# kspalaiologos/modern-rzip

Measured on AMD Instinct MI355X. Metric: rzip-stage GiB/s (mrzip -n), higher is better.
Workload: dtype u8; 1 GPU; tar-64G: rzip stage of mrzip -L7 on a 64 GiB synthetic tar (60 % text members, 25 % noise, 15 % exact duplicates, 512-byte aligned; BASELINE configs[2], the largest single-GPU configuration), one chunk per GPU, input resident in HBM; level=7, chunk_bytes_per_gpu=68719476736, streams=1, mode=streams

## Files before the change

### modern-rzip_amd/csrc/mrz_seq_deep.hip

```cpp
#ifndef MRZ_DEEP_WAVES
#define MRZ_DEEP_WAVES 8
#endif
#define MRZ_SEQ_WAVES MRZ_DEEP_WAVES
#include "mrz_seq_common.h"
#include <cstddef>

#ifndef MRZ_DEEP_LANES
#define MRZ_DEEP_LANES 256
#endif
#ifndef MRZ_DEEP_GROUP
#define MRZ_DEEP_GROUP 8
#endif
#define MRZ_DEEP_THREADS (64 * MRZ_DEEP_WAVES)
#ifdef __HIP_DEVICE_COMPILE__
#define MRZ_DEEP_WAIT() asm volatile("s_waitcnt vmcnt(0)" ::: "memory")
#else
#define MRZ_DEEP_WAIT() ((void)0)
#endif
#define MRZ_DEEP_MAP 2048
#define MRZ_DEEP_CW_WORDS 32
#define MRZ_DEEP_XW 192

enum { MRZ_DK_NONE = 255, MRZ_DK_EMPTY = 0, MRZ_DK_OVER = 1, MRZ_DK_DISPLACE = 2, MRZ_DK_EVICT = 3 };
#define MRZ_DF_INS 1
#define MRZ_DF_CPLX 2
#define MRZ_DF_STALE 4
#define MRZ_DF_FE2 8
#define MRZ_DS_COOP 1
#define MRZ_DS_CONFLICT 2
#define MRZ_DS_CULLED 4
#define MRZ_DS_NOCULL 8

struct mrz_deep_recs {
    int64_t q[MRZ_DEEP_LANES], t[MRZ_DEEP_LANES];
    int64_t occ_t[MRZ_DEEP_LANES], occ_off[MRZ_DEEP_LANES];
    int64_t old_t[MRZ_DEEP_LANES], old_t2[MRZ_DEEP_LANES];
    int64_t cp_scan[MRZ_DEEP_LANES];
    int64_t alt_old_t[MRZ_DEEP_LANES];
    int alt_w[MRZ_DEEP_LANES];
    int h[MRZ_DEEP_LANES], fe[MRZ_DEEP_LANES], w[MRZ_DEEP_LANES], h2[MRZ_DEEP_LANES], w2[MRZ_DEEP_LANES];
    unsigned short xw_seen[MRZ_DEEP_LANES];
    unsigned char kind[MRZ_DEEP_LANES], kind2[MRZ_DEEP_LANES], nsame[MRZ_DEEP_LANES], flags[MRZ_DEEP_LANES];
    unsigned char alt_kind[MRZ_DEEP_LANES];
    int same_slot[MRZ_DEEP_LANES][MRZ_SMAX];
    int64_t same_off[MRZ_DEEP_LANES][MRZ_SMAX];
    unsigned short raw[MRZ_DEEP_LANES][MRZ_SMAX];
};

struct mrz_deep_lds {
    mrz_lead lead;
    int ctl[16];
    int wsum[MRZ_DEEP_WAVES], wsum2[MRZ_DEEP_WAVES], wmin[MRZ_DEEP_WAVES], wmin2[MRZ_DEEP_WAVES], wmin3[MRZ_DEEP_WAVES];
    int n_rescan;
    mrz_deep_recs R;
    int idx[MRZ_DEEP_LANES];
    int cmin[MRZ_DEEP_LANES];
    int cpos[MRZ_DEEP_LANES];
    int xw_n;
    int xw_slot[MRZ_DEEP_XW];
    unsigned short rescan_list[MRZ_DEEP_LANES];
    unsigned smap_key[MRZ_DEEP_MAP];
    int smap_lane[MRZ_DEEP_MAP];
    unsigned long long tmap_key[MRZ_DEEP_MAP];
    int tmap_lane[MRZ_DEEP_MAP];
    mrz_u64 cw[MRZ_DEEP_CW_WORDS];
    int cwcum[MRZ_DEEP_CW_WORDS + 1];
#ifdef MRZ_SEQ_STATS
    int64_t stat[MRZ_ST_N], stat_unused[MRZ_ST_N];
#endif
    mrz_coop_lds coop;
};

__device__ __forceinline__ bool mrz_deep_ranges_meet(int a, int la, int b, int lb, int smask) {
    return la > 0 && lb > 0 && ((((b - a) & smask) < la) || (((a - b) & smask) < lb));
}

__device__ static unsigned mrz_deep_probe_raw(const uint8_t *__restrict__ buf, int64_t q, int64_t op, int64_t end) {
    if (op >= q) return 0;
    int64_t maxf = end - q;
    if (maxf < 0) maxf = 0;
    const int64_t last_ok = end + (MRZ_MIN_MATCH - 16);
    uint4 fa[4], fb[4], ba[4], bb[4];
#pragma unroll
    for (int j = 0; j < 4; j++) {
        int64_t pa = q + j * 16, pb = op + j * 16;
        pa = pa < last_ok ? pa : last_ok;
        pb = pb < last_ok ? pb : last_ok;
        fa[j] = mrz_ld16(buf + pa);
        fb[j] = mrz_ld16(buf + pb);
        int64_t ra = q - (j + 1) * 16, rb = op - (j + 1) * 16;
        ra = ra > 0 ? ra : 0;
        rb = rb > 0 ? rb : 0;
        ba[j] = mrz_ld16(buf + ra);
        bb[j] = mrz_ld16(buf + rb);
    }
    int rawf;
    {
        const int d0 = mrz_first_diff16_bf(fa[0], fb[0]), d1 = mrz_first_diff16_bf(fa[1], fb[1]);
        const int d2 = mrz_first_diff16_bf(fa[2], fb[2]), d3 = mrz_first_diff16_bf(fa[3], fb[3]);
        rawf = d0 < 16 ? d0 : 16 + (d1 < 16 ? d1 : 16 + (d2 < 16 ? d2 : 16 + d3));
// ... 220 lines not shown
                fe = (sb + fe_idx) & smask;
                fe2 = fe_idx < 63 && ((m_empty >> (fe_idx + 1)) & 1);
            }
        }
    }
    if (nsame > MRZ_SMAX) cplx = true;
    if (kind == MRZ_DK_EVICT && max_chain > MRZ_SMAX) cplx = true;
    int h2 = 0, w2 = -1, kind2 = MRZ_DK_NONE;
    int64_t old_t2 = 0;
    if (kind == MRZ_DK_DISPLACE && !cplx) {
        const int rank2 = mrz_ones_rank(occ_t);
        h2 = (int)(occ_t & C.slot_mask);
        int round2 = 0;
        bool done = false;
        for (int grp = 0; !done; grp++) {
            if (grp >= max_groups) {
                cplx = true;
                break;
            }
            mrz_slot e[MRZ_DEEP_GROUP];
            const int s0 = h2 + grp * (64 * MRZ_DEEP_GROUP) + lane;
#pragma unroll
            for (int g = 0; g < MRZ_DEEP_GROUP; g++) e[g] = tab[(s0 + g * 64) & smask];
#pragma unroll
            for (int g = 0; g < MRZ_DEEP_GROUP; g++) {
                if (done) continue;
                const int sb = s0 - lane + g * 64;
                const bool empty = (e[g].off | e[g].t) == 0;
                const bool due = !empty && (e[g].t & better) != better;
                const bool low = !empty && !due && mrz_ones_rank(e[g].t) < rank2;
                const mrz_u64 m_empty = __ballot(empty), m_due = __ballot(due), m_low = __ballot(low);
                const mrz_u64 m_stop = m_empty | m_due | m_low;
                const int ks = m_stop ? __ffsll((long long)m_stop) - 1 : 64;
                const int nq = __popcll(__ballot(!empty && !due && !low && e[g].t == occ_t) & mrz_low_mask(ks));
                if (round2 + nq >= max_chain) {
                    cplx = true;
                    done = true;
                } else if (ks < 64) {
                    if ((m_low >> ks) & 1)
                        cplx = true;
                    else {
                        w2 = (sb + ks) & smask;
                        kind2 = ((m_empty >> ks) & 1) ? MRZ_DK_EMPTY : MRZ_DK_OVER;
                        if (kind2 == MRZ_DK_OVER) old_t2 = mrz_bcast64(e[g].t, ks);
                    }
                    done = true;
                } else
                    round2 += nq;
            }
        }
    }
    const int ns = nsame < MRZ_SMAX ? nsame : MRZ_SMAX;
    if (ns > nsame0) {
        MRZ_WAVE_SYNC();
        if (lane >= nsame0 && lane < ns) S->R.raw[i][lane] = (unsigned short)mrz_deep_probe_raw(buf, q, S->R.same_off[i][lane], C.end);
    }
    if (lane == 0) {
        S->R.h[i] = h;
        S->R.fe[i] = fe;
        S->R.w[i] = w;
        S->R.kind[i] = (unsigned char)(kind < 0 ? MRZ_DK_NONE : kind);
        S->R.h2[i] = h2;
        S->R.w2[i] = w2;
        S->R.kind2[i] = (unsigned char)kind2;
        S->R.occ_t[i] = occ_t;
        S->R.occ_off[i] = occ_off;
        S->R.old_t[i] = old_t;
        S->R.old_t2[i] = old_t2;
        S->R.alt_w[i] = (cplx || kind == MRZ_DK_DISPLACE || kind == MRZ_DK_EVICT || insert_kept) ? -1 : alt_w;
        S->R.alt_kind[i] = (unsigned char)alt_kind;
        S->R.alt_old_t[i] = alt_old_t;
        S->R.nsame[i] = (unsigned char)ns;
        S->R.flags[i] = (unsigned char)((ins ? MRZ_DF_INS : 0) | (cplx ? MRZ_DF_CPLX : 0) | (fe2 ? MRZ_DF_FE2 : 0));
        if (!cont) {
            S->R.cp_scan[i] = clean_ptr;
            S->R.xw_seen[i] = (unsigned short)xw_n;
        }
    }
}

#ifndef MRZ_DEEP_SCANNERS
#define MRZ_DEEP_SCANNERS 63
#endif
#ifndef MRZ_DEEP_HELP_MIN
#define MRZ_DEEP_HELP_MIN 48
#endif

struct mrz_deep_shared {
    unsigned long long seq;
    unsigned long long quit;
    unsigned long long n_ok;
    unsigned long long xcc_plus1;
    unsigned long long pad0[12];
    long long nb, nscan, better, tag_mask, clean_ptr, xw_n;
    long long pad1[10];
    unsigned long long done;
    unsigned long long pad2[15];
    mrz_deep_recs R;
};

#ifdef __HIP_DEVICE_COMPILE__
#define MRZ_DEEP_ACQUIRE() __builtin_amdgcn_fence(__ATOMIC_ACQUIRE, "agent")
#define MRZ_DEEP_RELEASE() __builtin_amdgcn_fence(__ATOMIC_RELEASE, "agent")
#define MRZ_DEEP_XCC_ID() (__builtin_amdgcn_s_getreg(20 | (0 << 6) | (3 << 11)) & 15)
#else
#define MRZ_DEEP_ACQUIRE() ((void)0)
#define MRZ_DEEP_RELEASE() ((void)0)
#define MRZ_DEEP_XCC_ID() 0
#endif

__device__ __forceinline__ void mrz_deep_rec_copy(mrz_deep_recs *dst, const mrz_deep_recs *src, int i) {
    dst->occ_t[i] = src->occ_t[i];
    dst->occ_off[i] = src->occ_off[i];
    dst->old_t[i] = src->old_t[i];
    dst->old_t2[i] = src->old_t2[i];
    dst->cp_scan[i] = src->cp_scan[i];
    dst->alt_old_t[i] = src->alt_old_t[i];
    dst->alt_w[i] = src->alt_w[i];
    dst->alt_kind[i] = src->alt_kind[i];
    dst->h[i] = src->h[i];
    dst->fe[i] = src->fe[i];
    dst->w[i] = src->w[i];
    dst->h2[i] = src->h2[i];
    dst->w2[i] = src->w2[i];
    dst->xw_seen[i] = src->xw_seen[i];
    dst->kind[i] = src->kind[i];
    dst->kind2[i] = src->kind2[i];
    dst->flags[i] = src->flags[i];
    const int ns = src->nsame[i];
    dst->nsame[i] = (unsigned char)ns;
    for (int k = 0; k < ns; k++) {
        dst->same_slot[i][k] = src->same_slot[i][k];
        dst->same_off[i][k] = src->same_off[i][k];
        dst->raw[i][k] = src->raw[i][k];
    }
}


__device__ static void mrz_deep_scan_helper(const mrz_cfg &C, mrz_deep_lds *S, mrz_deep_shared *G, int tid, int lane, int wave) {
    if (tid == 0) {
        long long spins = 0;
        unsigned long long x = 0;
        while ((x = __hip_atomic_load(&G->xcc_plus1, __ATOMIC_RELAXED, __HIP_MEMORY_SCOPE_AGENT)) == 0 &&
               !__hip_atomic_load(&G->quit, __ATOMIC_RELAXED, __HIP_MEMORY_SCOPE_AGENT) && spins++ < (1ll << 24))
            __builtin_amdgcn_s_sleep(8);
        int ticket = -1;
        if (x != 0)
            ticket = (int)__hip_atomic_fetch_add(&G->n_ok, 1ull, __ATOMIC_RELAXED, __HIP_MEMORY_SCOPE_AGENT);
        S->ctl[0] = ticket;
    }
    __syncthreads();
    const int ticket = mrz_uni(S->ctl[0]);
    if (ticket < 0 || ticket >= MRZ_DEEP_SCANNERS) return;
    const int me = ticket + 1;
    unsigned long long seen = 0;
    while (true) {
        if (tid == 0) {
            long long spins = 0;
            unsigned long long sq = 0;
            int v = 1;
            while (true) {
                sq = __hip_atomic_load(&G->seq, __ATOMIC_RELAXED, __HIP_MEMORY_SCOPE_AGENT);
                if (sq != seen) break;
                if (__hip_atomic_load(&G->quit, __ATOMIC_RELAXED, __HIP_MEMORY_SCOPE_AGENT) || spins++ > MRZ_HELPER_SPIN_LIMIT) {
                    v = 0;
                    break;
                }
                __builtin_amdgcn_s_sleep(2);
            }
            MRZ_DEEP_ACQUIRE();
            S->ctl[1] = v;
            S->lead.p = (int64_t)sq;
        }
        __syncthreads();
        if (!mrz_uni(S->ctl[1])) return;
        seen = (unsigned long long)mrz_uni64(S->lead.p);
        const int nb = (int)G->nb, nscan = (int)G->nscan, xw_n = (int)G->xw_n;
        const int64_t better = G->better, tag_mask = G->tag_mask, clean_ptr = G->clean_ptr;
        int mine_n = 0;
        if (me < nscan) {
            for (int i = me + tid * nscan; i < nb; i += nscan * MRZ_DEEP_THREADS) {
                S->R.q[i] = G->R.q[i];
                S->R.t[i] = G->R.t[i];
            }
            __syncthreads();
            int k = 0;
            for (int i = me; i < nb; i += nscan, k++)
                if (k % MRZ_DEEP_WAVES == wave) mrz_deep_scan(C, S, i, better, tag_mask, clean_ptr, xw_n, lane);
            mine_n = k;
            __syncthreads();
            for (int i = me + tid * nscan; i < nb; i += nscan * MRZ_DEEP_THREADS) mrz_deep_rec_copy(&G->R, &S->R, i);
            MRZ_DEEP_WAIT();
        }
        __syncthreads();
        if (tid == 0 && mine_n) {
            MRZ_DEEP_RELEASE();
            __hip_atomic_fetch_add(&G->done, (unsigned long long)mine_n, __ATOMIC_RELEASE, __HIP_MEMORY_SCOPE_AGENT);
        }
    }
}

__device__ static __attribute__((noinline)) bool mrz_deep_coop(const mrz_cfg &C, mrz_lead &L, mrz_coop_lds *B, int64_t t,
                                                               int lane, int64_t *stat) {
    return mrz_seq_candidate(C, L, B, t, lane, stat);
}

__device__ static __attribute__((noinline)) bool mrz_deep_candidate_rec(const mrz_cfg &C, mrz_lead &L, mrz_deep_lds *S, int i, int *xw_n, int lane,
                                              int64_t *stat) {
    mrz_coop_lds *B = &S->coop;
    const int64_t q = mrz_uni64(S->R.q[i]), t = mrz_uni64(S->R.t[i]);
    const int ns = mrz_uni((int)S->R.nsame[i]);
    const int f = mrz_uni((int)S->R.flags[i]);
    int64_t mlen = 0, m_off = 0, m_rev = 0;
    L.p = q;
    if (ns) {
        if (lane < ns) {
            const int64_t op = S->R.same_off[i][lane];
            B->same_off[lane] = op;
            int64_t ml, rv;
            bool lng;
            mrz_lane_match_len(C.buf, q, op, C.end, L.last_match, &ml, &rv, &lng);
            B->pair_res[lane] = lng ? -1 : (int)((ml << 8) | rv);
        }
        MRZ_WAVE_SYNC();
        int xh = 0, xm = 0;
        if (!mrz_resolve_entries(C, L, B, q, ns, lane, stat, &mlen, &m_off, &m_rev, &xh, &xm)) return false;
        L.tag_hits += xh;
        L.tag_misses += xm;
    }
    int nx = *xw_n;
    if (f & MRZ_DF_INS) {
        const int kind = mrz_uni((int)S->R.kind[i]);
        L.inserts++;
        L.count++;
        int ws = mrz_uni(S->R.w[i]);
        if (kind == MRZ_DK_OVER)
            L.count--;
        else if (kind == MRZ_DK_EVICT) {
            L.count--;
            ws = mrz_uni(S->R.same_slot[i][(int)L.victim_round]);
            L.victim_round = L.victim_round + 1 == C.max_chain ? 0 : L.victim_round + 1;
        } else if (kind == MRZ_DK_DISPLACE) {
            const int w2 = mrz_uni(S->R.w2[i]);
            if (mrz_uni((int)S->R.kind2[i]) == MRZ_DK_OVER) L.count--;
            if (lane == 0) {
                mrz_slot oc;
                oc.off = S->R.occ_off[i];
                oc.t = S->R.occ_t[i];
                C.tab[w2] = oc;
                S->xw_slot[nx] = w2;
            }
            nx++;
        }
        if (lane == 0) {
            mrz_slot nw;
            nw.off = q;
            nw.t = t;
            C.tab[ws] = nw;
            S->xw_slot[nx] = ws;
        }
        nx++;
        if (L.count > C.limit) {
            MRZ_DEEP_WAIT();
            mrz_cull_one(C, L, lane);
            if (lane == 0) S->xw_slot[nx] = (int)L.clean_ptr;
            nx++;
        }
    }
    *xw_n = nx;
    return mrz_select_emit(C, L, mlen, m_off, m_rev, lane);
}

__device__ __forceinline__ int mrz_deep_incl(int v, int *ws, int lane, int wave, int *total) {
    const int incl = mrz_wave_incl_sum(v, lane);
    if (lane == 63) ws[wave] = incl;
    __syncthreads();
    int add = 0, tot = 0;
#pragma unroll
    for (int w = 0; w < MRZ_DEEP_WAVES; w++) {
        const int x = ws[w];
        tot += x;
        if (w < wave) add += x;
// ... 5 lines not shown
__device__ __forceinline__ int mrz_deep_first(bool flag, int *wm, int lane, int wave, int tid, int none) {
    const mrz_u64 m = __ballot(flag);
    if (lane == 0) wm[wave] = m ? wave * 64 + (__ffsll((long long)m) - 1) : none;
    __syncthreads();
    int r = none;
#pragma unroll
    for (int w = 0; w < MRZ_DEEP_WAVES; w++) r = wm[w] < r ? wm[w] : r;
    return r;
}

__global__ __launch_bounds__(MRZ_DEEP_THREADS) void mrz_seq_deep_kernel(mrz_seq_args a, mrz_deep_shared *G, int scanners) {
#ifdef MRZ_EMU_LDS_PER_BLOCK
    static mrz_deep_lds deep_all[1 + 15];
    mrz_deep_lds *S = &deep_all[(blockIdx.x / 8) % (1 + 15)];
#else
    __shared__ mrz_deep_lds deep;
    mrz_deep_lds *S = &deep;
#endif
    const int tid = (int)threadIdx.x;
    const int lane = tid & 63;
    const int wave = mrz_uni(tid >> 6);
    mrz_seq_state *st = a.st;
    if (st->finished || st->error) return;
    const int xcd = a.xcd & 7;
    const int bx = (int)blockIdx.x;
    const bool is_seq = bx == xcd;
#ifdef MRZ_EMU_LDS_PER_BLOCK
    const bool is_scanner = G != nullptr && !is_seq && bx % 8 == xcd && bx / 8 >= 1 && bx / 8 <= scanners && bx / 8 <= MRZ_DEEP_SCANNERS;
#else
    const bool is_scanner = G != nullptr && !is_seq && (bx < xcd ? bx : bx - 1) < scanners && scanners <= MRZ_DEEP_SCANNERS;
#endif
#if MRZ_HELPER_WGS > 0
    if (!is_seq && !is_scanner) {
        if (a.gmailbox) mrz_helper_wg(a.buf, (mrz_gmailbox *)a.gmailbox);
        return;
    }
#else
    if (!is_seq && !is_scanner) return;
#endif
    mrz_cfg C;
    C.buf = a.buf;
    C.tab = a.tab;
    C.events = a.events;
    C.st = st;
    C.end = st->end;
    C.limit = st->limit;
    C.max_chain = st->max_chain;
    C.slot_mask = st->slot_mask;
    C.nslots = st->slot_mask + 1;
    C.event_cap = st->event_cap;
    C.ev_base = st->ev_base;
    C.gmb = (mrz_gmailbox *)a.gmailbox;
    unsigned long long gseq = 0;
    C.gseq = &gseq;
    int gnw = 0;
    C.gnw = &gnw;
    C.n_helpers = a.n_helpers;
    int64_t farm_hint = 0;
    C.farm_hint = &farm_hint;
    int long_seen = 0;
    C.long_seen = &long_seen;
    C.mb = nullptr;
    C.mb_seq = nullptr;
    mrz_cands K;
    K.cand = a.cand;
    K.tile_off = a.tile_off;
    K.bitmap = a.bitmap;
    K.seg_start = st->seg_start;
    K.seg_end = st->seg_end;
    K.n = st->n_cand;
    if (is_scanner) {
        mrz_deep_scan_helper(C, S, G, tid, lane, wave);
        return;
    }
    if (K.seg_end <= K.seg_start) {
        if (tid == 0 && G) __hip_atomic_store(&G->quit, 1ull, __ATOMIC_RELAXED, __HIP_MEMORY_SCOPE_AGENT);
#if MRZ_HELPER_WGS > 0
        if (tid == 0 && C.gmb) mrz_g_storeu(&C.gmb->quit, 1ull);
#endif
        return;
    }
    if (tid == 0 && G) __hip_atomic_store(&G->xcc_plus1, (unsigned long long)MRZ_DEEP_XCC_ID() + 1ull, __ATOMIC_RELAXED, __HIP_MEMORY_SCOPE_AGENT);
    unsigned long long batch_seq = 0;
    const int64_t lim = (C.end < K.seg_end - 1) ? C.end : K.seg_end - 1;
    const int smask = (int)C.slot_mask;
    const int max_chain = (int)C.max_chain;
#ifdef MRZ_SEQ_STATS
    for (int k = tid; k < MRZ_ST_N; k += MRZ_DEEP_THREADS) S->stat[k] = 0;
    __syncthreads();
    int64_t *stat = tid == 0 ? S->stat : S->stat_unused;
#else
    int64_t *stat = nullptr;
#endif

    mrz_lead L;
    L.p = st->p;
    L.cur_p = st->cur_p;
    L.cur_ofs = st->cur_ofs;
    L.cur_len = st->cur_len;
    L.last_match = st->last_match;
    L.min_mask = st->min_mask;
    L.tag_mask = st->tag_mask;
    L.count = st->count;
    L.clean_ptr = st->clean_ptr;
    L.victim_round = st->victim_round;
    L.n_events = st->n_events;
    L.inserts = st->inserts;
    L.tag_hits = st->tag_hits;
    L.tag_misses = st->tag_misses;
    L.last_len = 0;
    L.mbytes = 0;
    const int64_t hint_p0 = L.p, hint_ev0 = L.n_events;

    int64_t ci;
    {
        int64_t pos = L.p + 1;
        if (pos < K.seg_start) pos = K.seg_start;
        ci = mrz_cand_lower_bound(K, pos, lane);
    }
    bool ok = true;
    PROF_T0();
#ifdef MRZ_SEQ_PROFILE
    const int64_t launch_t0 = (int64_t)__builtin_amdgcn_s_memtime();
#endif
    ST_ADD(MRZ_ST_D_LAUNCHES, 1);
    while (ok && ci < K.n && L.p < lim) {
        PROF_T0R();
        const int64_t better = (L.min_mask << 1) | 1;
        const bool loose = L.tag_mask != better;
        int64_t my_q = 0, my_t = 0;
        bool live = false;
        if (ci + tid < K.n) {
            const mrz_cand c = K.cand[ci + tid];
            my_q = c.off;
            my_t = c.t;
            live = c.off > L.p && c.off <= lim && (c.t & L.min_mask) == L.min_mask;
        }
        int total;
        const int incl = mrz_deep_incl(live ? 1 : 0, S->wsum, lane, wave, &total);
        const int at = incl - 1;
        if (live && at < MRZ_DEEP_LANES) {
            S->R.q[at] = my_q;
            S->R.t[at] = my_t;
            S->idx[at] = (int)(ci + tid);
        }
        const int nb = total < MRZ_DEEP_LANES ? total : MRZ_DEEP_LANES;
        int64_t n_examined = K.n - ci < MRZ_DEEP_THREADS ? K.n - ci : MRZ_DEEP_THREADS;
        __syncthreads();
        if (total > MRZ_DEEP_LANES) n_examined = (int64_t)S->idx[MRZ_DEEP_LANES - 1] + 1 - ci;
        if (nb == 0) {
            ci += n_examined;
            __syncthreads();
            continue;
        }
        ST_ADD(MRZ_ST_D_BATCHES, 1);
        ST_ADD(MRZ_ST_D_LANES, nb);
        PROF_ADD(MRZ_ST_D_T_FORM);
        if (!loose) {
            int nscan = 1;
            if (G && nb >= MRZ_DEEP_HELP_MIN) {
                int nh = (int)mrz_uni64((int64_t)__hip_atomic_load(&G->n_ok, __ATOMIC_RELAXED, __HIP_MEMORY_SCOPE_AGENT));
                if (nh > MRZ_DEEP_SCANNERS) nh = MRZ_DEEP_SCANNERS;
                if (nh > scanners) nh = scanners;
                nscan = 1 + nh;
            }
            int helper_lanes = 0;
            if (nscan > 1) {
                if (tid < nb) {
                    G->R.q[tid] = S->R.q[tid];
                    G->R.t[tid] = S->R.t[tid];
                }
                if (tid == 0) {
                    G->nb = nb;
                    G->nscan = nscan;
                    G->better = better;
                    G->tag_mask = L.tag_mask;
                    G->clean_ptr = L.clean_ptr;
                    G->xw_n = 0;
                    __hip_atomic_store(&G->done, 0ull, __ATOMIC_RELAXED, __HIP_MEMORY_SCOPE_AGENT);
                }
                MRZ_DEEP_WAIT();
                __syncthreads();
                batch_seq++;
                if (tid == 0) {
                    MRZ_DEEP_RELEASE();
                    __hip_atomic_store(&G->seq, batch_seq, __ATOMIC_RELEASE, __HIP_MEMORY_SCOPE_AGENT);
                }
                helper_lanes = nb - (nb + nscan - 1) / nscan;
            }
            {
                int k = 0;
                for (int i = 0; i < nb; i += nscan, k++)
                    if (k % MRZ_DEEP_WAVES == wave) mrz_deep_scan(C, S, i, better, L.tag_mask, L.clean_ptr, 0, lane);
            }
            if (nscan > 1) {
                if (tid == 0) {
                    long long spins = 0;
                    while (__hip_atomic_load(&G->done, __ATOMIC_ACQUIRE, __HIP_MEMORY_SCOPE_AGENT) < (unsigned long long)helper_lanes &&
                           spins++ < (1ll << 26))
                        __builtin_amdgcn_s_sleep(1);
                    S->ctl[6] = spins < (1ll << 26) ? 1 : 0;
                    MRZ_DEEP_ACQUIRE();
                }
                __syncthreads();
                if (!mrz_uni(S->ctl[6])) {
                    if (tid == 0) C.st->error = 7;
                    ok = false;
                } else if (tid < nb && tid % nscan != 0)
                    mrz_deep_rec_copy(&S->R, &G->R, tid);
            }
        }
        __syncthreads();
        PROF_ADD(MRZ_ST_D_T_SCAN);
        for (int k = tid; k < MRZ_DEEP_MAP; k += MRZ_DEEP_THREADS) {
            S->smap_key[k] = 0u;
            S->smap_lane[k] = 0x7fffffff;
            S->tmap_key[k] = 0ull;
            S->tmap_lane[k] = 0x7fffffff;
        }
        __syncthreads();
        int next = 0;
        bool cut = false;
        int xw_n = 0;
        while (next < nb && !cut && ok) {
            const int i = tid;
            const bool mine = i >= next && i < nb;
            const int round_start = next;
            int coop_lane = -1;
            bool use_record = false;
            if (loose || L.cur_len > 0) {
                coop_lane = next;
            } else {
                const int64_t cw_base = L.clean_ptr;
                const bool load_cw = L.count + (nb - next) > C.limit;
                constexpr int CW_PER_WAVE = (MRZ_DEEP_CW_WORDS + MRZ_DEEP_WAVES - 1) / MRZ_DEEP_WAVES;
                mrz_slot cwe[CW_PER_WAVE];
#pragma unroll
                for (int b = 0; b < CW_PER_WAVE; b++) {
                    cwe[b].off = 0;
                    cwe[b].t = 0;
                    const int wi = b * MRZ_DEEP_WAVES + wave;
                    const int64_t slot = cw_base + (int64_t)wi * 64 + lane;
                    if (load_cw && wi < MRZ_DEEP_CW_WORDS && slot < C.nslots) cwe[b] = C.tab[slot];
                }
                const int f = mine ? S->R.flags[i] : 0;
                const bool ins = mine && (f & MRZ_DF_INS), cplx = mine && (f & MRZ_DF_CPLX);
                const int kind = mine ? S->R.kind[i] : MRZ_DK_NONE, kind2 = mine ? S->R.kind2[i] : MRZ_DK_NONE;
                const int64_t q = mine ? S->R.q[i] : 0, t = mine ? S->R.t[i] : 0;
                const int w = mine ? S->R.w[i] : -1, w2 = mine ? S->R.w2[i] : -1, fe = mine ? S->R.fe[i] : -1;
                const int h = mine ? S->R.h[i] : 0, h2 = mine ? S->R.h2[i] : 0;
                const int64_t occ_t = mine ? S->R.occ_t[i] : 0;
                const bool wr_w = ins && !cplx && (kind == MRZ_DK_EMPTY || kind == MRZ_DK_OVER || kind == MRZ_DK_DISPLACE);
                const bool wr_w2 = ins && !cplx && kind == MRZ_DK_DISPLACE;
                if (ins && !cplx) {
                    if (wr_w) mrz_deep_smap_put(S, w, i);
                    if (wr_w2) mrz_deep_smap_put(S, w2, i);
                    mrz_deep_tmap_put(S, t, i);
                    if (kind == MRZ_DK_OVER) mrz_deep_tmap_put(S, S->R.old_t[i], i);
                    if (kind == MRZ_DK_DISPLACE) {
                        mrz_deep_tmap_put(S, occ_t, i);
                        if (kind2 == MRZ_DK_OVER) mrz_deep_tmap_put(S, S->R.old_t2[i], i);
                    }
                }
                __syncthreads();
                int res = 0, res_x = -1;
                int w_e = w, kind_e = kind, fe_e = fe;
                if (mine && !cplx && !(f & MRZ_DF_STALE) && kind != MRZ_DK_DISPLACE) {
                    const int m_t = mrz_deep_tmap_get(S, t);
                    const int m_fe = mrz_deep_smap_get(S, fe);
                    const int m_w = wr_w ? mrz_deep_smap_get(S, w) : 0x7fffffff;
                    const bool c_w = wr_w && m_w < i, c_fe = m_fe < i;
                    if (m_t >= i && (c_w || c_fe)) {
                        bool can = true;
                        const int aw = S->R.alt_w[i], ak = S->R.alt_kind[i];
                        if (c_w) {
                            const int x = m_w;
                            res_x = x;
                            const int kx = S->R.kind[x];
                            can = aw >= 0 && S->R.w[x] == w && (kx == MRZ_DK_EMPTY || kx == MRZ_DK_OVER) &&
                                  mrz_ones_rank(S->R.t[x]) >= mrz_ones_rank(t);
                            res |= 1;
                            if (kind == MRZ_DK_EMPTY) res |= 2;
                        }
                        if (c_fe && !(res & 2)) {
                            can = can && (f & MRZ_DF_FE2) && !((res & 1) && ak == MRZ_DK_EMPTY);
                            res |= 2;
                        }
                        if (!can) res = 0;
                    }
                    if (res & 1) {
                        w_e = S->R.alt_w[i];
                        kind_e = S->R.alt_kind[i];
// ... 293 lines not shown
                                             : mrz_deep_coop(C, L, &S->coop, t, lane, stat);
                        ST_ADD(MRZ_ST_D_COOP, 1);
                        ST_ADD(MRZ_ST_D_COOP_REC, rec ? 1 : 0);
                        const bool same_masks = L.min_mask == mm0 && L.tag_mask == tm0;
                        const int nwr = rec ? 0 : mrz_uni(S->coop.n_written);
                        const int64_t cs = rec ? -1 : mrz_uni64(S->coop.cull_slot);
                        const bool room = nx + nwr + 1 <= MRZ_DEEP_XW;
                        if (rec)
                            nx = nx_rec;
                        else if (okc && same_masks && room && !loose) {
                            if (lane < nwr) S->xw_slot[nx + lane] = (int)S->coop.pend_h[lane];
                            nx += nwr;
                            if (cs >= 0) {
                                if (lane == 0) S->xw_slot[nx] = (int)cs;
                                nx++;
                            }
                        }
                        verdict = !okc ? 3 : ((same_masks && (room || loose) && L.p >= q) ? 1 : 2);
                        if (!(loose && verdict == 1)) break;
                        int j = cl + 1;
                        while (j < nb && mrz_uni64(S->R.q[j]) <= L.p) j++;
                        if (j >= nb) break;
                        cl = j;
                    }
                    if (lane == 0) {
                        S->lead = L;
                        S->ctl[0] = verdict;
                        S->ctl[5] = nx;
                    }
                    MRZ_DEEP_WAIT();
                }
                __syncthreads();
                L = S->lead;
                xw_n = mrz_uni(S->ctl[5]);
                const int v = mrz_uni(S->ctl[0]);
                if (v == 3) ok = false;
                if (v == 2) cut = true;
                {
                    const int i = tid;
                    const int nf = mrz_deep_first(i > coop_lane && i < nb && S->R.q[i] > L.p, S->wmin3, lane, wave, tid, nb);
                    next = nf;
                }
                PROF_ADD(MRZ_ST_D_T_COOP);
            }
        }
        if (ok) {
            if (cut || L.p > mrz_uni64(S->R.q[nb - 1])) {
                int64_t pos = L.p + 1;
                if (pos < K.seg_start) pos = K.seg_start;
                ci = mrz_cand_lower_bound(K, pos, lane);
            } else
                ci += n_examined;
        }
        __syncthreads();
    }
    if (ok && ci >= K.n && L.p < lim) L.p = lim;
#ifdef MRZ_SEQ_PROFILE
    stat[MRZ_ST_D_T_TOTAL] += (int64_t)__builtin_amdgcn_s_memtime() - launch_t0;
#endif
    if (tid == 0) {
        if (G) __hip_atomic_store(&G->quit, 1ull, __ATOMIC_RELAXED, __HIP_MEMORY_SCOPE_AGENT);
#if MRZ_HELPER_WGS > 0
        if (C.gmb) mrz_g_storeu(&C.gmb->quit, 1ull);
#endif
        st->p = L.p;
        st->cur_p = L.cur_p;
        st->cur_ofs = L.cur_ofs;
        st->cur_len = L.cur_len;
        st->last_match = L.last_match;
        st->min_mask = L.min_mask;
        st->tag_mask = L.tag_mask;
        st->count = L.count;
        st->clean_ptr = L.clean_ptr;
        st->victim_round = L.victim_round;
        st->n_events = L.n_events;
        st->inserts = L.inserts;
        st->tag_hits = L.tag_hits;
        st->tag_misses = L.tag_misses;
        st->finished = L.p >= C.end ? 1 : 0;
        st->hint_positions = L.p - hint_p0;
        st->hint_events = L.n_events - hint_ev0;
        st->hint_matched = L.mbytes;
#ifdef MRZ_SEQ_STATS
        for (int k = 0; k < MRZ_ST_N; k++) st->prof[k] += stat[k];
#endif
    }
}

extern "C" hipError_t mrz_launch_sequencer_deep(hipStream_t stream, const uint8_t *buf, mrz_slot *tab, const mrz_cand *cand,
                                                const int *tile_off, const mrz_u64 *bitmap, mrz_event *events,
                                                mrz_seq_state *st, void *gmailbox, int n_helpers, int xcd, void *deep_shared,
                                                int scanners) {
    mrz_seq_args a;
    a.buf = buf;
    a.tab = tab;
    a.cand = cand;
    a.tile_off = tile_off;
    a.bitmap = bitmap;
    a.events = events;
    a.st = st;
    a.gmailbox = gmailbox;
    a.xcd = xcd & 7;
    a.deep_bits = 0;
#if MRZ_HELPER_WGS == 0
    n_helpers = 0;
#endif
    if (n_helpers > MRZ_HELPER_WGS) n_helpers = MRZ_HELPER_WGS;
    if (n_helpers < 0 || !gmailbox) n_helpers = 0;
    a.n_helpers = n_helpers;
    if (gmailbox) {
        hipError_t e = hipMemsetAsync(gmailbox, 0, sizeof(mrz_gmailbox), stream);
        if (e != hipSuccess) return e;
    }
    if (scanners < 0 || !deep_shared) scanners = 0;
    if (scanners > MRZ_DEEP_SCANNERS) scanners = MRZ_DEEP_SCANNERS;
    unsigned grid = (unsigned)(1 + a.n_helpers);
    if (grid < (unsigned)(a.xcd + 1)) grid = (unsigned)(a.xcd + 1);
#ifdef MRZ_EMU_LDS_PER_BLOCK
    if (scanners > 0) {
        grid = (unsigned)(8 * scanners + a.xcd + 1);
        emu::request_coresident();
    }
#else
    if (scanners > a.n_helpers / 2) scanners = a.n_helpers / 2;
    while (scanners > 0 && grid < (unsigned)(scanners + 2)) scanners--;
#endif
    if (deep_shared) {
        hipError_t e = hipMemsetAsync(deep_shared, 0, offsetof(mrz_deep_shared, R), stream);
        if (e != hipSuccess) return e;
    }
    hipLaunchKernelGGL(mrz_seq_deep_kernel, dim3(grid), dim3(MRZ_DEEP_THREADS), 0, stream, a, (mrz_deep_shared *)deep_shared,
                       scanners);
    return hipGetLastError();
}

extern "C" size_t mrz_seq_deep_shared_size(void) { return sizeof(mrz_deep_shared); }
```

### modern-rzip_amd/csrc/mrz_seq_stats.h

```cpp
#pragma once
#include "mrz_common.h"

#define MRZ_SEQ_STATS_LIST(X) \
    X(BATCHES, "batches") X(FORMED, "formed") X(COMMITTED, "committed") X(SEGMENTS, "segments") \
    X(EMITS, "emits") X(BACKJUMP, "backjump") X(REWALK, "rewalk") X(LONGRES, "longres") X(SEQ, "seq_cands") \
    X(CUT_CPLX, "cut_cplx") X(CUT_OVERFLOW, "cut_overflow") X(SKIPOUT, "skipout") X(CONF0, "conf0") \
    X(PAIRS, "pairs") X(T_FORM, "t_form") X(T_WALK, "t_walk") X(T_CONF, "t_conf") X(T_PAIRS, "t_pairs") \
    X(T_LOOP, "t_loop") X(T_REWALK, "t_rewalk") X(T_LONG, "t_long") X(T_SEQ, "t_seq") X(FARMED, "farmed") \
    X(L_POST, "l_post") X(L_STRIPE, "l_stripe") X(L_BWD, "l_bwd") X(L_WAIT, "l_wait") X(L_ROUNDS, "l_rounds") \
    X(F_POST, "f_post") X(F_WAIT, "f_wait") X(F_FOLD, "f_fold") X(S_TAB, "s_tab") X(S_PAIR, "s_pair") \
    X(S_INS, "s_ins") X(OVL, "ovl") X(OVL_OK, "ovl_ok") X(X_WALK, "x_walk") X(X_CASC, "x_casc") \
    X(X_POOL, "x_pool") X(X_WIN, "x_win") X(X_SAME, "x_same") X(C_WIN, "c_win") X(C_EVICT, "c_evict") \
    X(C_DEEP, "c_deep") X(C_MANY, "c_many") X(C_FAIL, "c_fail") X(C_TIE, "c_tie") X(C_NW, "c_nw") \
    X(T_OVL, "t_ovl") X(H_PRE, "h_pre") X(H_CAND, "h_cand") X(H_POST, "h_post") X(T_SCAN, "t_scan") \
    X(T_FOLD, "t_fold") X(T_COMMIT, "t_commit") X(REPREP, "reprep") X(W_STALE, "w_stale") X(W_DROP, "w_drop") \
    X(RESET, "reset") X(T_TURN, "t_turn") X(T_PREP, "t_prep") X(T_PRECOMMIT, "t_precommit") X(E_MASK, "e_mask") \
    X(E_CULL, "e_cull") X(E_XW, "e_xw") X(E_INWIN, "e_inwin") X(E_WINDOW, "e_window") X(E_BULK, "e_bulk") \
    X(E_MORE, "e_more") X(T_PC_CW, "t_pc_cw") X(T_PC_LOG, "t_pc_log") X(T_PC_BEST, "t_pc_best") \
    X(T_PC_BULK, "t_pc_bulk") X(T_TURNWORK, "t_turnwork") X(T_SNAP, "t_snap") X(REBULK, "rebulk") \
     \
    X(BATCH_LANES, "batch_lanes") X(CUT_LONG, "cut_long") X(CUT_WALK, "cut_walk") \
    X(CUT_CONFLICT, "cut_conflict") X(CUT_CULL, "cut_cull") X(BATCH_EMITS, "batch_emits") \
    X(CUT_CASCADE, "cut_cascade") X(BATCH_FORMED, "batch_formed") X(T_WALK2, "t_walk2") X(T_SCANS, "t_scans") \
    X(T_CONFLICT, "t_conflict") X(T_WINDOW, "t_window") \
     \
    X(D_BATCHES, "d_batches") X(D_LANES, "d_lanes") X(D_ROUNDS, "d_rounds") X(D_RESCANNED, "d_rescanned") \
    X(D_COOP, "d_coop") X(D_T_FORM, "d_t_form") X(D_T_SCAN, "d_t_scan") X(D_T_COMMIT, "d_t_commit") \
    X(D_T_RESCAN, "d_t_rescan") X(D_T_TOTAL, "d_t_total") X(D_LAUNCHES, "d_launches") X(D_T_COOP, "d_t_coop") \
    X(D_COOP_REC, "d_coop_rec") X(D_RESOLVED, "d_resolved") X(D_S_COOP, "d_s_coop") \
    X(D_S_CONFLICT, "d_s_conflict") X(D_S_CULLED, "d_s_culled") X(D_S_NOCULL, "d_s_nocull") \
    X(D_S_STALE, "d_s_stale") X(D_C_OVER_ALT, "d_c_over_alt") X(D_C_OVER_NOALT, "d_c_over_noalt") \
    X(D_C_EMPTY, "d_c_empty") X(D_C_DISPLACE, "d_c_displace") X(D_C_OTHER, "d_c_other")

#define MRZ_ST_ENUM(id, name) MRZ_ST_##id,
enum { MRZ_SEQ_STATS_LIST(MRZ_ST_ENUM) MRZ_ST_N };
#undef MRZ_ST_ENUM
static_assert(MRZ_ST_N <= (int)(sizeof(((mrz_seq_state *)0)->prof) / sizeof(int64_t)), "mrz_seq_state.prof holds the counters");
```

Baseline: 6.362 GiB/s.

## Hand off deep-scan records as packed 16-byte granules with stamped jobs and unfenced counters

Scanner helpers now pack each scanned record into an array-of-structs of 16-byte granules and write it right after scanning, using buffer stores with a cache-coherence bit instead of a field-by-field struct-of-arrays copy after a barrier. The leader pulls those granules back with vectorised loads. Job parameters go out as a single stamped 16-byte word so helpers can detect a stale job, and the done counter becomes cumulative, which lets the agent-scope release/acquire fences be dropped on both sides. This is meant to cut handoff latency and fence cost per batch. It relies on the SC1 buffer semantics for coherence in place of explicit fences, which is a correctness risk if those semantics do not hold. Optional profiling counters are also added.

```diff
diff --git a/modern-rzip_amd/csrc/mrz_seq_deep.hip b/modern-rzip_amd/csrc/mrz_seq_deep.hip
--- a/modern-rzip_amd/csrc/mrz_seq_deep.hip
+++ b/modern-rzip_amd/csrc/mrz_seq_deep.hip
@@ -16,6 +16,20 @@
 #define MRZ_DEEP_WAIT() asm volatile("s_waitcnt vmcnt(0)" ::: "memory")
 #else
 #define MRZ_DEEP_WAIT() ((void)0)
+#endif
+#ifdef MRZ_SEQ_PROFILE
+#define DPROF_T0() int64_t dprof_t0 = (int64_t)__builtin_amdgcn_s_memtime()
+#define DPROF_T0R() dprof_t0 = (int64_t)__builtin_amdgcn_s_memtime()
+#define DPROF_ADD(acc)                                               \
+    do {                                                             \
+        const int64_t now__ = (int64_t)__builtin_amdgcn_s_memtime(); \
+        (acc) += now__ - dprof_t0;                                   \
+        dprof_t0 = now__;                                            \
+    } while (0)
+#else
+#define DPROF_T0()
+#define DPROF_T0R()
+#define DPROF_ADD(acc)
 #endif
 #define MRZ_DEEP_MAP 2048
 #define MRZ_DEEP_CW_WORDS 32
@@ -402,9 +416,34 @@
 #ifndef MRZ_DEEP_SCANNERS
 #define MRZ_DEEP_SCANNERS 63
 #endif
+#define MRZ_DEEP_STAMP_RETRIES (1 << 20)
 #ifndef MRZ_DEEP_HELP_MIN
 #define MRZ_DEEP_HELP_MIN 48
 #endif
+
+#define MRZ_DEEP_REC_HDR 5
+#define MRZ_DEEP_REC_GRANULES (MRZ_DEEP_REC_HDR + MRZ_SMAX)
+struct mrz_deep_rec_ent {
+    int64_t same_off;
+    int same_slot;
+    unsigned short raw, pad;
+};
+struct __attribute__((aligned(16))) mrz_deep_rec {
+    int64_t occ_t, occ_off;
+    int64_t old_t, old_t2;
+    int64_t cp_scan, alt_old_t;
+    int alt_w, h, fe, w;
+    int h2, w2;
+    unsigned short xw_seen;
+    unsigned char kind, kind2, nsame, flags, alt_kind, pad;
+    mrz_deep_rec_ent ent[MRZ_SMAX];
+};
+static_assert(sizeof(mrz_deep_rec_ent) == 16 && sizeof(mrz_deep_rec) == 16 * MRZ_DEEP_REC_GRANULES, "records travel as 16-byte granules");
+
+struct __attribute__((aligned(16))) mrz_deep_stamp {
+    unsigned long long job_seq;
+    int nb, nscan;
+};
 
 struct mrz_deep_shared {
     unsigned long long seq;
@@ -412,12 +451,17 @@
     unsigned long long n_ok;
     unsigned long long xcc_plus1;
     unsigned long long pad0[12];
-    long long nb, nscan, better, tag_mask, clean_ptr, xw_n;
+    mrz_deep_stamp stamp;
+    long long better, tag_mask, clean_ptr, xw_n;
     long long pad1[10];
     unsigned long long done;
     unsigned long long pad2[15];
-    mrz_deep_recs R;
+    int64_t q[MRZ_DEEP_LANES], t[MRZ_DEEP_LANES];
+    mrz_deep_rec rec[MRZ_DEEP_LANES];
 };
+static_assert(offsetof(mrz_deep_shared, stamp) % 128 == 0 && offsetof(mrz_deep_shared, done) % 128 == 0 &&
+                  offsetof(mrz_deep_shared, q) % 128 == 0 && offsetof(mrz_deep_shared, rec) % 16 == 0,
+              "the polled words, the job and the counter have lines of their own; granules are aligned");
 
 #ifdef __HIP_DEVICE_COMPILE__
 #define MRZ_DEEP_ACQUIRE() __builtin_amdgcn_fence(__ATOMIC_ACQUIRE, "agent")
@@ -429,33 +473,136 @@
 #define MRZ_DEEP_XCC_ID() 0
 #endif
 
-__device__ __forceinline__ void mrz_deep_rec_copy(mrz_deep_recs *dst, const mrz_deep_recs *src, int i) {
-    dst->occ_t[i] = src->occ_t[i];
-    dst->occ_off[i] = src->occ_off[i];
-    dst->old_t[i] = src->old_t[i];
-    dst->old_t2[i] = src->old_t2[i];
-    dst->cp_scan[i] = src->cp_scan[i];
-    dst->alt_old_t[i] = src->alt_old_t[i];
-    dst->alt_w[i] = src->alt_w[i];
-    dst->alt_kind[i] = src->alt_kind[i];
-    dst->h[i] = src->h[i];
-    dst->fe[i] = src->fe[i];
-    dst->w[i] = src->w[i];
-    dst->h2[i] = src->h2[i];
-    dst->w2[i] = src->w2[i];
-    dst->xw_seen[i] = src->xw_seen[i];
-    dst->kind[i] = src->kind[i];
-    dst->kind2[i] = src->kind2[i];
-    dst->flags[i] = src->flags[i];
-    const int ns = src->nsame[i];
-    dst->nsame[i] = (unsigned char)ns;
-    for (int k = 0; k < ns; k++) {
-        dst->same_slot[i][k] = src->same_slot[i][k];
-        dst->same_off[i][k] = src->same_off[i][k];
-        dst->raw[i][k] = src->raw[i][k];
-    }
-}
-
+__device__ static __attribute__((noinline)) uint4 mrz_deep_rec_granule(const mrz_deep_recs *R, int i, int g) {
+    if (g < 3) {
+        const int64_t a = g == 0 ? R->occ_t[i] : g == 1 ? R->old_t[i] : R->cp_scan[i];
+        const int64_t b = g == 0 ? R->occ_off[i] : g == 1 ? R->old_t2[i] : R->alt_old_t[i];
+        return make_uint4((uint32_t)(uint64_t)a, (uint32_t)((uint64_t)a >> 32), (uint32_t)(uint64_t)b, (uint32_t)((uint64_t)b >> 32));
+    }
+    if (g == 3) return make_uint4((uint32_t)R->alt_w[i], (uint32_t)R->h[i], (uint32_t)R->fe[i], (uint32_t)R->w[i]);
+    if (g == 4)
+        return make_uint4((uint32_t)R->h2[i], (uint32_t)R->w2[i],
+                          (uint32_t)R->xw_seen[i] | ((uint32_t)R->kind[i] << 16) | ((uint32_t)R->kind2[i] << 24),
+                          (uint32_t)R->nsame[i] | ((uint32_t)R->flags[i] << 8) | ((uint32_t)R->alt_kind[i] << 16));
+    const int k = g - MRZ_DEEP_REC_HDR;
+    const int64_t o = R->same_off[i][k];
+    return make_uint4((uint32_t)(uint64_t)o, (uint32_t)((uint64_t)o >> 32), (uint32_t)R->same_slot[i][k], (uint32_t)R->raw[i][k]);
+}
+
+__device__ __forceinline__ void mrz_deep_rec_ungranule(mrz_deep_recs *R, int i, int g, uint4 v, int nsame) {
+    const int64_t a = (int64_t)(((uint64_t)v.y << 32) | v.x), b = (int64_t)(((uint64_t)v.w << 32) | v.z);
+    if (g == 0) {
+        R->occ_t[i] = a;
+        R->occ_off[i] = b;
+    } else if (g == 1) {
+        R->old_t[i] = a;
+        R->old_t2[i] = b;
+    } else if (g == 2) {
+        R->cp_scan[i] = a;
+        R->alt_old_t[i] = b;
+    } else if (g == 3) {
+        R->alt_w[i] = (int)v.x;
+        R->h[i] = (int)v.y;
+        R->fe[i] = (int)v.z;
+        R->w[i] = (int)v.w;
+    } else if (g == 4) {
+        R->h2[i] = (int)v.x;
+        R->w2[i] = (int)v.y;
+        R->xw_seen[i] = (unsigned short)(v.z & 0xffffu);
+        R->kind[i] = (unsigned char)((v.z >> 16) & 0xffu);
+        R->kind2[i] = (unsigned char)(v.z >> 24);
+        R->nsame[i] = (unsigned char)(v.w & 0xffu);
+        R->flags[i] = (unsigned char)((v.w >> 8) & 0xffu);
+        R->alt_kind[i] = (unsigned char)((v.w >> 16) & 0xffu);
+    } else if (g - MRZ_DEEP_REC_HDR < nsame) {
+        const int k = g - MRZ_DEEP_REC_HDR;
+        R->same_off[i][k] = a;
+        R->same_slot[i][k] = (int)v.z;
+        R->raw[i][k] = (unsigned short)(v.w & 0xffffu);
+    }
+}
+
+#if defined(__HIP_DEVICE_COMPILE__) && !defined(MRZ_DEEP_HANDOFF_FENCED)
+#define MRZ_DEEP_SC1 16
+typedef uint32_t mrz_v4u __attribute__((ext_vector_type(4)));
+struct mrz_deep_recmem {
+    __amdgpu_buffer_rsrc_t rsrc;
+};
+__device__ __forceinline__ mrz_deep_recmem mrz_deep_recmem_of(mrz_deep_shared *G) {
+    mrz_deep_recmem m;
+    m.rsrc = __builtin_amdgcn_make_buffer_rsrc((void *)(uintptr_t)mrz_uni64((int64_t)(uintptr_t)G->rec), 0, (int)sizeof(G->rec), 0x00020000);
+    return m;
+}
+__device__ __forceinline__ void mrz_deep_granule_store(const mrz_deep_recmem &m, unsigned off, uint4 v) {
+    mrz_v4u x = {v.x, v.y, v.z, v.w};
+    __builtin_amdgcn_raw_buffer_store_b128(x, m.rsrc, (int)off, 0, MRZ_DEEP_SC1);
+}
+__device__ __forceinline__ uint4 mrz_deep_granule_load(const mrz_deep_recmem &m, bool take, unsigned off, int soff) {
+    const mrz_v4u x = __builtin_amdgcn_raw_buffer_load_b128(m.rsrc, (int)(take ? off : 0x40000000u), soff, MRZ_DEEP_SC1);
+    return make_uint4(x[0], x[1], x[2], x[3]);
+}
+#else
+struct mrz_deep_recmem {
+    char *base;
+};
+__device__ __forceinline__ mrz_deep_recmem mrz_deep_recmem_of(mrz_deep_shared *G) {
+    mrz_deep_recmem m;
+    m.base = (char *)G->rec;
+    return m;
+}
+__device__ __forceinline__ void mrz_deep_granule_store(const mrz_deep_recmem &m, unsigned off, uint4 v) {
+    *(uint4 *)(m.base + off) = v;
+}
+__device__ __forceinline__ uint4 mrz_deep_granule_load(const mrz_deep_recmem &m, bool take, unsigned off, int soff) {
+    return take ? *(const uint4 *)(m.base + off + soff) : make_uint4(0, 0, 0, 0);
+}
+#endif
+
+__device__ __forceinline__ void mrz_deep_rec_send(const mrz_deep_recmem &m, const mrz_deep_lds *S, int i, int lane) {
+    MRZ_WAVE_SYNC();
+    const int ng = MRZ_DEEP_REC_HDR + mrz_uni((int)S->R.nsame[i]);
+    if (lane < ng) mrz_deep_granule_store(m, (unsigned)(i * (int)sizeof(mrz_deep_rec) + lane * 16), mrz_deep_rec_granule(&S->R, i, lane));
+}
+
+#define MRZ_DEEP_REC_FIRST (MRZ_DEEP_REC_HDR + 1)
+#define MRZ_DEEP_FETCH_PER (MRZ_DEEP_THREADS / MRZ_DEEP_REC_FIRST)
+__device__ __forceinline__ void mrz_deep_recs_fetch(mrz_deep_shared *G, mrz_deep_lds *S, int nb, int nscan, int tid) {
+    const mrz_deep_recmem m = mrz_deep_recmem_of(G);
+    constexpr int NLD = (MRZ_DEEP_LANES + MRZ_DEEP_FETCH_PER - 1) / MRZ_DEEP_FETCH_PER;
+    constexpr int CH = 5;
+#ifdef __HIP_DEVICE_COMPILE__
+    asm volatile("" : "+v"(tid));
+#endif
+    const int i0 = tid / MRZ_DEEP_REC_FIRST, g = tid - i0 * MRZ_DEEP_REC_FIRST;
+    const unsigned off0 = (unsigned)(i0 * (int)sizeof(mrz_deep_rec) + g * 16);
+    bool take[NLD];
+#pragma unroll
+    for (int j = 0; j < NLD; j++) {
+        const int i = i0 + j * MRZ_DEEP_FETCH_PER;
+        take[j] = i0 < MRZ_DEEP_FETCH_PER && i < nb && i % nscan != 0;
+    }
+    uint4 v[NLD];
+#pragma unroll
+    for (int j = 0; j < NLD; j++) {
+        v[j] = mrz_deep_granule_load(m, take[j], off0, j * MRZ_DEEP_FETCH_PER * (int)sizeof(mrz_deep_rec));
+    }
+#pragma unroll
+    for (int j = 0; j < NLD; j++)
+        if (take[j]) mrz_deep_rec_ungranule(&S->R, i0 + j * MRZ_DEEP_FETCH_PER, g, v[j], MRZ_SMAX);
+    __syncthreads();
+    const int ns = (tid < nb && tid % nscan != 0) ? (int)S->R.nsame[tid] : 0;
+    for (int k0 = 1; __ballot(k0 < ns) != 0; k0 += CH) {
+        const unsigned offe = (unsigned)(tid * (int)sizeof(mrz_deep_rec) + (MRZ_DEEP_REC_HDR + k0) * 16);
+        uint4 e[CH];
+#pragma unroll
+        for (int c = 0; c < CH; c++) {
+            e[c] = mrz_deep_granule_load(m, k0 + c < ns, offe, c * 16);
+        }
+#pragma unroll
+        for (int c = 0; c < CH; c++)
+            if (k0 + c < ns) mrz_deep_rec_ungranule(&S->R, tid, MRZ_DEEP_REC_HDR + k0 + c, e[c], ns);
+    }
+}
 
 __device__ static void mrz_deep_scan_helper(const mrz_cfg &C, mrz_deep_lds *S, mrz_deep_shared *G, int tid, int lane, int wave) {
     if (tid == 0) {
@@ -473,7 +620,13 @@
     const int ticket = mrz_uni(S->ctl[0]);
     if (ticket < 0 || ticket >= MRZ_DEEP_SCANNERS) return;
     const int me = ticket + 1;
+    const mrz_deep_recmem recmem = mrz_deep_recmem_of(G);
     unsigned long long seen = 0;
+    int retries = 0;
+#ifdef MRZ_SEQ_PROFILE
+    int64_t hprof[4] = {0, 0, 0, 0};
+#endif
+    DPROF_T0();
     while (true) {
         if (tid == 0) {
             long long spins = 0;
@@ -481,43 +634,71 @@
             int v = 1;
             while (true) {
                 sq = __hip_atomic_load(&G->seq, __ATOMIC_RELAXED, __HIP_MEMORY_SCOPE_AGENT);
-                if (sq != seen) break;
+                if (sq != seen && retries == 0) break;
                 if (__hip_atomic_load(&G->quit, __ATOMIC_RELAXED, __HIP_MEMORY_SCOPE_AGENT) || spins++ > MRZ_HELPER_SPIN_LIMIT) {
                     v = 0;
                     break;
                 }
+                if (sq != seen) break;
                 __builtin_amdgcn_s_sleep(2);
             }
+            DPROF_T0R();
             MRZ_DEEP_ACQUIRE();
+            MRZ_DEEP_WAIT();
             S->ctl[1] = v;
             S->lead.p = (int64_t)sq;
         }
         __syncthreads();
-        if (!mrz_uni(S->ctl[1])) return;
-        seen = (unsigned long long)mrz_uni64(S->lead.p);
-        const int nb = (int)G->nb, nscan = (int)G->nscan, xw_n = (int)G->xw_n;
+        if (!mrz_uni(S->ctl[1])) break;
+        DPROF_ADD(hprof[0]);
+        const unsigned long long sq = (unsigned long long)mrz_uni64(S->lead.p);
+        const uint4 sv = *(const uint4 *)&G->stamp;
+        const unsigned long long job_seq = (unsigned long long)mrz_uni64((int64_t)(((unsigned long long)sv.y << 32) | sv.x));
+        const int nb = mrz_uni((int)sv.z), nscan = mrz_uni((int)sv.w);
+        const int xw_n = (int)G->xw_n;
         const int64_t better = G->better, tag_mask = G->tag_mask, clean_ptr = G->clean_ptr;
+        if (job_seq != sq) {
+            if (++retries > MRZ_DEEP_STAMP_RETRIES) break;
+            __syncthreads();
+            continue;
+        }
+        retries = 0;
+        seen = sq;
         int mine_n = 0;
         if (me < nscan) {
             for (int i = me + tid * nscan; i < nb; i += nscan * MRZ_DEEP_THREADS) {
-                S->R.q[i] = G->R.q[i];
-                S->R.t[i] = G->R.t[i];
+                S->R.q[i] = G->q[i];
+                S->R.t[i] = G->t[i];
             }
             __syncthreads();
+            DPROF_ADD(hprof[1]);
             int k = 0;
             for (int i = me; i < nb; i += nscan, k++)
-                if (k % MRZ_DEEP_WAVES == wave) mrz_deep_scan(C, S, i, better, tag_mask, clean_ptr, xw_n, lane);
+                if (k % MRZ_DEEP_WAVES == wave) {
+                    mrz_deep_scan(C, S, i, better, tag_mask, clean_ptr, xw_n, lane);
+                    mrz_deep_rec_send(recmem, S, i, lane);
+                }
             mine_n = k;
+            MRZ_DEEP_WAIT();
+#ifdef MRZ_SEQ_PROFILE
             __syncthreads();
-            for (int i = me + tid * nscan; i < nb; i += nscan * MRZ_DEEP_THREADS) mrz_deep_rec_copy(&G->R, &S->R, i);
-            MRZ_DEEP_WAIT();
+            DPROF_ADD(hprof[2]);
+#endif
         }
         __syncthreads();
         if (tid == 0 && mine_n) {
+#ifdef MRZ_DEEP_HANDOFF_FENCED
             MRZ_DEEP_RELEASE();
-            __hip_atomic_fetch_add(&G->done, (unsigned long long)mine_n, __ATOMIC_RELEASE, __HIP_MEMORY_SCOPE_AGENT);
-        }
-    }
+            MRZ_DEEP_WAIT();
+#endif
+            __hip_atomic_fetch_add(&G->done, (unsigned long long)mine_n, __ATOMIC_RELAXED, __HIP_MEMORY_SCOPE_AGENT);
+            DPROF_ADD(hprof[3]);
+        }
+    }
+#ifdef MRZ_SEQ_PROFILE
+    if (tid == 0 && ticket == 0)
+        for (int k = 0; k < 4; k++) C.st->prof[MRZ_ST_DH_T_ACQ + k] += hprof[k];
+#endif
 }
 
 __device__ static __attribute__((noinline)) bool mrz_deep_coop(const mrz_cfg &C, mrz_lead &L, mrz_coop_lds *B, int64_t t,
@@ -689,6 +870,7 @@
     }
     if (tid == 0 && G) __hip_atomic_store(&G->xcc_plus1, (unsigned long long)MRZ_DEEP_XCC_ID() + 1ull, __ATOMIC_RELAXED, __HIP_MEMORY_SCOPE_AGENT);
     unsigned long long batch_seq = 0;
+    unsigned long long done_target = 0;
     const int64_t lim = (C.end < K.seg_end - 1) ? C.end : K.seg_end - 1;
     const int smask = (int)C.slot_mask;
     const int max_chain = (int)C.max_chain;
@@ -763,6 +945,7 @@
         ST_ADD(MRZ_ST_D_BATCHES, 1);
         ST_ADD(MRZ_ST_D_LANES, nb);
         PROF_ADD(MRZ_ST_D_T_FORM);
+        DPROF_T0();
         if (!loose) {
             int nscan = 1;
             if (G && nb >= MRZ_DEEP_HELP_MIN) {
@@ -773,27 +956,28 @@
             }
             int helper_lanes = 0;
             if (nscan > 1) {
+                batch_seq++;
                 if (tid < nb) {
-                    G->R.q[tid] = S->R.q[tid];
-                    G->R.t[tid] = S->R.t[tid];
+                    G->q[tid] = S->R.q[tid];
+                    G->t[tid] = S->R.t[tid];
                 }
                 if (tid == 0) {
-                    G->nb = nb;
-                    G->nscan = nscan;
+                    *(uint4 *)&G->stamp = make_uint4((uint32_t)batch_seq, (uint32_t)(batch_seq >> 32), (uint32_t)nb, (uint32_t)nscan);
                     G->better = better;
                     G->tag_mask = L.tag_mask;
                     G->clean_ptr = L.clean_ptr;
                     G->xw_n = 0;
-                    __hip_atomic_store(&G->done, 0ull, __ATOMIC_RELAXED, __HIP_MEMORY_SCOPE_AGENT);
                 }
                 MRZ_DEEP_WAIT();
                 __syncthreads();
-                batch_seq++;
                 if (tid == 0) {
                     MRZ_DEEP_RELEASE();
-                    __hip_atomic_store(&G->seq, batch_seq, __ATOMIC_RELEASE, __HIP_MEMORY_SCOPE_AGENT);
+                    MRZ_DEEP_WAIT();
+                    __hip_atomic_store(&G->seq, batch_seq, __ATOMIC_RELAXED, __HIP_MEMORY_SCOPE_AGENT);
                 }
                 helper_lanes = nb - (nb + nscan - 1) / nscan;
+                done_target += (unsigned long long)helper_lanes;
+                DPROF_ADD(stat[MRZ_ST_D_T_POST]);
             }
             {
                 int k = 0;
@@ -801,20 +985,28 @@
                     if (k % MRZ_DEEP_WAVES == wave) mrz_deep_scan(C, S, i, better, L.tag_mask, L.clean_ptr, 0, lane);
             }
             if (nscan > 1) {
+                DPROF_ADD(stat[MRZ_ST_D_T_OWN]);
                 if (tid == 0) {
                     long long spins = 0;
-                    while (__hip_atomic_load(&G->done, __ATOMIC_ACQUIRE, __HIP_MEMORY_SCOPE_AGENT) < (unsigned long long)helper_lanes &&
-                           spins++ < (1ll << 26))
+                    while (__hip_atomic_load(&G->done, __ATOMIC_RELAXED, __HIP_MEMORY_SCOPE_AGENT) < done_target && spins++ < (1ll << 26))
                         __builtin_amdgcn_s_sleep(1);
                     S->ctl[6] = spins < (1ll << 26) ? 1 : 0;
+#ifdef MRZ_DEEP_HANDOFF_FENCED
                     MRZ_DEEP_ACQUIRE();
+                    MRZ_DEEP_WAIT();
+#endif
                 }
                 __syncthreads();
+                DPROF_ADD(stat[MRZ_ST_D_T_WAIT]);
                 if (!mrz_uni(S->ctl[6])) {
                     if (tid == 0) C.st->error = 7;
                     ok = false;
-                } else if (tid < nb && tid % nscan != 0)
-                    mrz_deep_rec_copy(&S->R, &G->R, tid);
+                } else
+                    mrz_deep_recs_fetch(G, S, nb, nscan, tid);
+#ifdef MRZ_SEQ_PROFILE
+                __syncthreads();
+                DPROF_ADD(stat[MRZ_ST_D_T_COPYIN]);
+#endif
             }
         }
         __syncthreads();
@@ -1274,7 +1466,8 @@
         st->hint_events = L.n_events - hint_ev0;
         st->hint_matched = L.mbytes;
 #ifdef MRZ_SEQ_STATS
-        for (int k = 0; k < MRZ_ST_N; k++) st->prof[k] += stat[k];
+        for (int k = 0; k < MRZ_ST_N; k++)
+            if (k < MRZ_ST_DH_T_ACQ || k > MRZ_ST_DH_T_OUT) st->prof[k] += stat[k];
 #endif
     }
 }
@@ -1318,7 +1511,7 @@
     while (scanners > 0 && grid < (unsigned)(scanners + 2)) scanners--;
 #endif
     if (deep_shared) {
-        hipError_t e = hipMemsetAsync(deep_shared, 0, offsetof(mrz_deep_shared, R), stream);
+        hipError_t e = hipMemsetAsync(deep_shared, 0, offsetof(mrz_deep_shared, q), stream);
         if (e != hipSuccess) return e;
     }
     hipLaunchKernelGGL(mrz_seq_deep_kernel, dim3(grid), dim3(MRZ_DEEP_THREADS), 0, stream, a, (mrz_deep_shared *)deep_shared,
diff --git a/modern-rzip_amd/csrc/mrz_seq_stats.h b/modern-rzip_amd/csrc/mrz_seq_stats.h
--- a/modern-rzip_amd/csrc/mrz_seq_stats.h
+++ b/modern-rzip_amd/csrc/mrz_seq_stats.h
@@ -30,7 +30,10 @@
     X(D_COOP_REC, "d_coop_rec") X(D_RESOLVED, "d_resolved") X(D_S_COOP, "d_s_coop") \
     X(D_S_CONFLICT, "d_s_conflict") X(D_S_CULLED, "d_s_culled") X(D_S_NOCULL, "d_s_nocull") \
     X(D_S_STALE, "d_s_stale") X(D_C_OVER_ALT, "d_c_over_alt") X(D_C_OVER_NOALT, "d_c_over_noalt") \
-    X(D_C_EMPTY, "d_c_empty") X(D_C_DISPLACE, "d_c_displace") X(D_C_OTHER, "d_c_other")
+    X(D_C_EMPTY, "d_c_empty") X(D_C_DISPLACE, "d_c_displace") X(D_C_OTHER, "d_c_other") \
+     \
+    X(D_T_POST, "d_t_post") X(D_T_OWN, "d_t_own") X(D_T_WAIT, "d_t_wait") X(D_T_COPYIN, "d_t_copyin") \
+    X(DH_T_ACQ, "dh_t_acq") X(DH_T_JOB, "dh_t_job") X(DH_T_SCAN, "dh_t_scan") X(DH_T_OUT, "dh_t_out")
 
 #define MRZ_ST_ENUM(id, name) MRZ_ST_##id,
 enum { MRZ_SEQ_STATS_LIST(MRZ_ST_ENUM) MRZ_ST_N };
```

After: 6.764 GiB/s (median of 6 runs). +6.3%, better.
